# AlexZou14/Wave-Mamba

Hardware: AMD Instinct MI355X
Metric: UHD (3840x2160) images/sec fwd (higher is better)
Workload: dtype f32; 1 GPU; Wave-Mamba UHD-LL inference config (wf=32, n_l=[1,2,4], n_h=[1,1,2]), 1x3x2160x3840 reflect-padded to 2176x3840, seeded random init, one image per GPU per step, replicas (no collective); one forward at a time, its down-path high-frequency branches on side streams: True

## Files before the change

### include/wavemamba_hip.h

```cpp
#ifndef WAVEMAMBA_HIP_H
#define WAVEMAMBA_HIP_H

#include <stddef.h>
#include <stdint.h>

#ifdef __cplusplus
extern "C" {
#endif

#define WM_OK 0
#define WM_EINVAL (-1)
#define WM_ENULL (-2)
#define WM_EALIGN (-3)
#define WM_EWORKSPACE (-4)
#define WM_EUNSUPPORTED (-5)
#define WM_EHIP (-6)

#define WM_F32 0
#define WM_BF16 1

int wm_abi_version(void);
const char* wm_build_id(void);
const char* wm_strerror(int code);

// ... 52 lines not shown
                       int C, int plane_dtype, void* stream);
int wm_lfss_out_fwd(const void* fc, const float* tok1, const float* conv3_weight, const float* conv3_bias,
                    const float* skip_scale2, float* out, int out_nchw, int B, int64_t L, int C, int plane_dtype,
                    void* stream);
int wm_lfss_in_conv_fwd(const float* tok, int tok_nchw, const float* ln_w, const float* ln_b, float ln_eps,
                        const float* in_proj_weight, const float* conv_weight, const float* conv_bias, float* xc,
                        int B, int H, int W, int C, int plane_dtype, void* stream);
int wm_lfss_in_conv_band_rows(int B, int H, int W);
int wm_lfss_out_conv_fwd(const void* f, const float* conv2_weight, const float* conv2_bias, const float* tok1,
                         const float* conv3_weight, const float* conv3_bias, const float* skip_scale2, float* out,
                         int out_nchw, int B, int H, int W, int C, int plane_dtype, void* stream);

int wm_layernorm2d_fwd(const float* x, const float* weight, const float* bias, float eps, float* y,
                       int B, int64_t L, int C, void* stream);

size_t wm_gram_workspace_bytes(int B, int C, int64_t L);
int wm_gram_fwd(const float* X, const float* Y, float* G, float* nx, float* ny, void* workspace,
                size_t workspace_bytes, int B, int C, int64_t L, void* stream);

int wm_dwconv3x3_wgrad(const float* x, const float* gy, float* dW, float* db, int B, int C, int H, int W,
                       void* stream);
int wm_layernorm2d_bwd(const float* x, const float* weight, const float* gy, float eps, float* gx,
                       float* dweight, float* dbias, int B, int64_t L, int C, void* stream);


int wm_conv2d_select(int mode);
size_t wm_conv2d_wfrag_bytes(int Cout, int Cin, int ks);
int wm_conv2d_prep(const float* weight, void* wfrag, int Cout, int Cin, int ks, void* stream);
int wm_conv2d_ln_fwd(const float* x, const float* ln_weight, const float* ln_bias, float ln_eps, const void* wfrag, const float* bias,
                     const float* residual, float* y, int B, int Cin, int Cout, int H, int W, void* stream);
int wm_dwconv_conv1x1_fwd(const float* x, int64_t x_batch_stride, const float* dw_weight, const float* dw_bias, int act,
                          const void* wfrag, const float* bias, const float* residual, float* y, int B, int C, int Cout, int H,
                          int W, void* stream);
int wm_conv2d_f16_steps(const float* x, const float* weight, const float* bias, float* y, float* amax, void* wfrag, int B, int Cin,
                        int Cout, int H, int W, int ks, int dgrad, void* stream);
int wm_conv2d_fwd(const float* xa, const float* xb, const int* xb_index, const void* wfrag, const float* bias,
                  const float* gate, const float* residual, float* y, int B, int Ca, int Cb, int Cb_src, int Cout,
                  int H, int W, int ks, void* stream);
int wm_conv2d_gated_fwd(const float* xa, const float* xb, const int* xb_index, const void* wfrag3, const void* wfrag1,
                        const float* bias1, float* y, int B, int Ca, int Cb, int Cb_src, int Cout, int H, int W,
                        void* stream);
int wm_conv2d_dwt_fwd(const void* img, const void* wfrag, const float* bias, void* ll, void* hl, void* lh, void* hh, int B, int Cin,
                      int Cout, int H, int W, int dtype, void* stream);
int wm_idwt_conv2d_fwd(const void* low, const void* high, const void* wfrag, const float* bias, const float* residual, float* y, int B,
                       int Cin, int Cout, int H, int W, int dtype, void* stream);

size_t wm_ss2d_core_bwd_workspace_bytes(int B, int D, int H, int W, int N, int R);
int wm_ss2d_core_bwd(const float* x, const float* x_proj_weight, const float* dt_projs_weight,
                     const float* dt_projs_bias, const float* A_logs, const float* Ds, const float* dy_row_fwd,
                     const float* dy_row_rev, const float* dy_col_fwd, const float* dy_col_rev, float* dx,
                     float* dx_proj_weight, float* ddt_projs_weight, float* ddt_projs_bias, float* dA_logs, float* dDs,
                     void* workspace, size_t workspace_bytes, int B, int D, int H, int W, int N, int R, void* stream);

int wm_layernorm_tok_fwd(const float* x, const float* weight, const float* bias, float eps, float* y, int64_t T, int C,
                         void* stream);
int wm_layernorm_tok_bwd(const float* x, const float* weight, const float* gy, float eps, float* gx, float* dweight,
                         float* dbias, int64_t T, int C, void* stream);

int wm_image_pre_u8(const uint8_t* image, float* out, int h, int w, int Hp, int Wp, int swap_rb, void* stream);
int wm_image_post_u8(const float* in, uint8_t* image, int h, int w, int Hp, int Wp, int swap_rb, void* stream);

int wm_paired_patches_u8(const int64_t* table, float* lq, float* gt, int B, int P, int swap_rb, void* stream);

int wm_linear_wgrad(const float* gy, const float* x, float* dW, int64_t T, int O, int I, void* stream);
size_t wm_conv2d_wgrad_workspace_bytes(int B, int Cin, int Cout, int H, int W, int ks);
int wm_conv2d_wgrad(const float* gy, const float* x, float* dW, float* db, void* workspace, size_t workspace_bytes, int B, int Cin,
// ... 52 lines not shown
```

### wave_mamba_amd/_lib.py

```python
import ctypes
import os

HERE = os.path.dirname(os.path.abspath(__file__))
LIB_PATH = os.environ.get("WAVEMAMBA_HIP_LIB") or os.path.join(HERE, "libwavemamba_hip.so")

WM_F32, WM_BF16 = 0, 1
WM_OK, WM_EINVAL, WM_ENULL, WM_EALIGN, WM_EWORKSPACE, WM_EUNSUPPORTED, WM_EHIP = 0, -1, -2, -3, -4, -5, -6
WM_PROF_NKERNELS = 20
ABI_VERSION = 34

_c = ctypes
_p, _i, _i64, _sz = _c.c_void_p, _c.c_int, _c.c_int64, _c.c_size_t

SIGNATURES = {
    "wm_abi_version": (_i, []),
    "wm_build_id": (_c.c_char_p, []),
    "wm_strerror": (_c.c_char_p, [_i]),
    "wm_dwt2d_fwd": (_i, [_p] * 5 + [_i] * 5 + [_p]),
    "wm_dwt2d_bwd": (_i, [_p] * 5 + [_i] * 5 + [_p]),
    "wm_idwt2d_fwd": (_i, [_p] * 4 + [_i64] * 4 + [_p] + [_i] * 5 + [_p]),
    "wm_idwt2d_bwd": (_i, [_p] * 5 + [_i64] * 4 + [_i] * 5 + [_p]),
    "wm_selscan_fwd_workspace_bytes": (_sz, [_i] * 5),
    "wm_selscan_fwd": (_i, [_p] * 10 + [_p, _sz] + [_i] * 6 + [_p]),
    "wm_selscan_bwd_workspace_bytes": (_sz, [_i] * 5),
# ... 20 lines not shown
    "wm_dwconv3x3_wgrad": (_i, [_p] * 4 + [_i] * 4 + [_p]),
    "wm_layernorm2d_bwd": (_i, [_p, _p, _p, _c.c_float, _p, _p, _p, _i, _i64, _i, _p]),
    "wm_dwconv3x3_fwd": (_i, [_p] * 4 + [_i] * 6 + [_p]),
    "wm_layernorm_tok_fwd": (_i, [_p, _p, _p, _c.c_float, _p, _i64, _i, _p]),
    "wm_layernorm_tok_bwd": (_i, [_p, _p, _p, _c.c_float, _p, _p, _p, _i64, _i, _p]),
    "wm_image_pre_u8": (_i, [_p, _p, _i, _i, _i, _i, _i, _p]),
    "wm_image_post_u8": (_i, [_p, _p, _i, _i, _i, _i, _i, _p]),
    "wm_paired_patches_u8": (_i, [_p, _p, _p, _i, _i, _i, _p]),
    "wm_linear_wgrad": (_i, [_p, _p, _p, _i64, _i, _i, _p]),
    "wm_conv2d_wgrad_workspace_bytes": (_sz, [_i] * 6),
    "wm_conv2d_wgrad": (_i, [_p, _p, _p, _p, _p, _sz] + [_i] * 6 + [_p]),
    "wm_plane_sums": (_i, [_p, _p, _i, _i, _i, _i, _p]),
    "wm_psnr_ssim_y_workspace_bytes": (_sz, [_i] * 4),
    "wm_psnr_ssim_y_u8": (_i, [_p, _p] + [_i64] * 4 + [_i] * 5 + [_p, _p, _sz, _p]),
    "wm_y_channel_u8": (_i, [_p] + [_i64] * 4 + [_i] * 4 + [_p, _p]),
    "wm_l1_mean_fwd": (_i, [_p, _p, _p, _i64, _p]),
    "wm_l1_mean_bwd": (_i, [_p, _p, _p, _p, _i64, _p]),
    "wm_ssim_workspace_bytes": (_sz, [_i64, _i, _i]),
    "wm_ssim_mean_fwd": (_i, [_p] * 8 + [_sz, _i64, _i, _i, _p]),
    "wm_ssim_mean_bwd": (_i, [_p] * 7 + [_i64, _i, _i, _p]),
    "wm_gate_fwd": (_i, [_p] * 3 + [_i, _i] + [_i64] * 4 + [_p]),
    "wm_gate_bwd": (_i, [_p] * 5 + [_i, _i] + [_i64] * 6 + [_p]),
    "wm_scale_add_fwd": (_i, [_p] * 4 + [_i, _i, _i64, _p]),
    "wm_scale_add_bwd": (_i, [_p] * 5 + [_i, _i, _i64, _p]),
    "wm_match_index": (_i, [_p, _p, _p, _p, _i, _i, _p]),
    "wm_attn_fold": (_i, [_p] * 6 + [_i, _i, _i, _p]),
    "wm_skff_workspace_bytes": (_sz, [_i, _i]),
    "wm_skff_fwd": (_i, [_p] * 7 + [_p, _sz] + [_i] * 5 + [_p]),
    "wm_conv2d_wfrag_bytes": (_sz, [_i, _i, _i]),
    "wm_conv2d_prep": (_i, [_p, _p, _i, _i, _i, _p]),
    "wm_conv2d_fwd": (_i, [_p] * 8 + [_i] * 8 + [_p]),
    "wm_conv2d_ln_fwd": (_i, [_p, _p, _p, _c.c_float, _p, _p, _p, _p] + [_i] * 5 + [_p]),
    "wm_dwconv_conv1x1_fwd": (_i, [_p, _i64, _p, _p, _i, _p, _p, _p, _p] + [_i] * 5 + [_p]),
    "wm_patchify_conv_fwd": (_i, [_p] * 4 + [_i] * 6 + [_p]),
    "wm_conv2d_f16_steps": (_i, [_p] * 6 + [_i] * 7 + [_p]),
    "wm_conv2d_gated_fwd": (_i, [_p] * 7 + [_i] * 7 + [_p]),
    "wm_conv2d_dwt_fwd": (_i, [_p] * 7 + [_i] * 6 + [_p]),
    "wm_idwt_conv2d_fwd": (_i, [_p] * 6 + [_i] * 6 + [_p]),
    "wm_conv2d_select": (_i, [_i]),
    "wm_prof_enable": (None, [ctypes.c_uint]),
    "wm_prof_collect": (_i, [_c.POINTER(_i), _c.POINTER(_c.c_double)]),
    "wm_event_synchronize_relaxed": (_i, [_p]),
    "wm_zero_arena_register": (_i, [_p, _c.c_size_t]),
    "wm_zero_arena_unregister": (_i, [_p]),
}

_lib = None


class WaveMambaHipError(RuntimeError):
    pass


def load():
    global _lib
    if _lib is not None:
        return _lib
    if not os.path.exists(LIB_PATH):
        raise WaveMambaHipError(
            f"{LIB_PATH} not found: build it with `python -c 'import __graft_entry__ as g; g.build()'` "
            "(hipcc --offload-arch=gfx950). The Wave-Mamba hot path has no CPU or PyTorch fallback.")
    try:
        lib = ctypes.CDLL(LIB_PATH)
    except OSError as e:
        raise WaveMambaHipError(f"cannot load {LIB_PATH}: {e}") from e
    for name, (res, args) in SIGNATURES.items():
# ... 24 lines not shown
```

### wave_mamba_amd/archs/wavemamba_arch.py

```python
import math

import os

import torch
import torch.nn as nn
import torch.nn.functional as F

try:
    from .. import ops as _hip_ops
    from ..registry import ARCH_REGISTRY
except ImportError:
    import wave_mamba_amd.ops as _hip_ops
    from basicsr.utils.registry import ARCH_REGISTRY


class _OpsBackend:
    impl = _hip_ops


def _op(name):
    return getattr(_OpsBackend.impl, name, None)


def _needs_grad(module, *tensors):
# ... 44 lines not shown
        y = conv(x)
    if gate is not None:
        if train and _op("gate_act") and ops.gate_supported(gate, y):
            y = ops.gate_act(gate, y, "sigmoid")
        else:
            y = y * torch.sigmoid(gate)
    if residual is not None:
        y = y + residual
    return y


def _ps_conv(ps, img):
    ops = _OpsBackend.impl
    r, conv = ps[0].downscale_factor, ps[1]
    if _op("patchify_conv") and ops.patchify_conv_supported(img, conv.weight, r) and not _needs_grad(conv, img):
        return ops.patchify_conv(img, conv.weight, conv.bias, r)
    return _conv(conv, ps[0](img))


def _ln_conv(norm, conv, x):
    if norm is None:
        return _conv(conv, x)
    ops = _OpsBackend.impl
    if (_op("conv2d_ln") and ops.conv2d_ln_supported(x, conv.weight) and not _needs_grad(conv, x)
            and not _needs_grad(norm, x)):
        return ops.conv2d_ln(x, norm.weight, norm.bias, norm.eps, conv.weight, conv.bias)
    return _conv(conv, norm(x))


def _dw_pw_fused(x, dw_weight, pw_weight):
    ops = _OpsBackend.impl
    return bool(_op("dwconv_conv1x1") and ops.dwconv_conv1x1_supported(x, dw_weight, pw_weight)
                and _hip_ops._fuse_dw_pw_map(x.shape[0], x.shape[2], x.shape[3]))


def _conv_dwt_fused(conv, img):
    ops = _OpsBackend.impl
    return bool(_op("conv2d_dwt") and ops.conv2d_dwt_supported(img, conv.weight) and not _needs_grad(conv, img)
                and _hip_ops._fuse_conv_dwt_map(img.shape[0], img.shape[2], img.shape[3]))


def _conv_dwt(conv, img):
    if _conv_dwt_fused(conv, img):
        return _OpsBackend.impl.conv2d_dwt(img, conv.weight, conv.bias)
    return _conv(conv, img)


def _iwt_conv_fused(net, conv, low, out_like):
    ops = _OpsBackend.impl
    return bool(_op("iwt_conv2d") and ops.iwt_conv2d_supported(low, conv.weight) and not _needs_grad(net, low, out_like)
                and _hip_ops._fuse_iwt_conv_map(out_like.shape[0], out_like.shape[2], out_like.shape[3]))


def _cat_gathered(x, x2=None, x2_index=None):
    if x2 is None:
        return x
    if x2_index is not None:
        x2 = torch.gather(x2, 1, x2_index.long()[:, :, None, None].expand(-1, -1, x2.shape[2], x2.shape[3]))
    return torch.cat([x, x2], dim=1)


class DWT(nn.Module):

    def forward(self, x):
        return _OpsBackend.impl.dwt_init(x)

# ... 292 lines not shown
class Matching_transformation(nn.Module):
    def __init__(self, dim=32, match_factor=1, ffn_expansion_factor=1, bias=True):
        super().__init__()
        self.num_matching = int(dim / match_factor)
        self.channel = dim
        self.matching = Matching(dim=dim, match_factor=match_factor)
        self.paconv = PAConv(dim * 2)

    def forward(self, x, perception):
        idx = nearest_candidate_index(x.flatten(2), perception.flatten(2), self.num_matching)
        return self.paconv(x, perception, idx)


class FeedForward(nn.Module):

    def __init__(self, dim=32, match_factor=4, ffn_expansion_factor=1, bias=True, ffn_matching=True):
        super().__init__()
        self.num_matching = int(dim / match_factor)
        self.channel = dim
        self.matching = ffn_matching
        hidden = int(dim * ffn_expansion_factor)
        self.project_in = nn.Sequential(
            nn.Conv2d(dim, hidden, 1, bias=bias),
            nn.Conv2d(hidden, dim, kernel_size=3, stride=1, padding=1, groups=dim, bias=bias))
        if self.matching is True:
            self.matching_transformation = Matching_transformation(
                dim=dim, match_factor=match_factor, ffn_expansion_factor=ffn_expansion_factor, bias=bias)
        self.project_out = nn.Sequential(
            nn.Conv2d(dim, hidden, kernel_size=3, stride=1, padding=1, groups=dim, bias=bias),
            nn.GELU(),
            nn.Conv2d(hidden, dim, 1, bias=bias))

    def forward(self, x, perception, residual=None, norm=None):
        y = _dwconv(self.project_in[1], _ln_conv(norm, self.project_in[0], x))
        if perception is not None:
            y = self.matching_transformation(y, perception)
        dw, pw = self.project_out[0], self.project_out[2]
        if _dw_pw_fused(y, dw.weight, pw.weight) and not _needs_grad(dw, y, residual) and not _needs_grad(pw):
            return _OpsBackend.impl.dwconv_conv1x1(y, dw.weight, dw.bias, "gelu", pw.weight, pw.bias, residual=residual)
        return _conv(pw, _dwconv(dw, y, act="gelu"), residual=residual)


class CMTAttention(nn.Module):

    def __init__(self, dim, num_heads, match_factor=4, ffn_expansion_factor=1, scale_factor=8, bias=True,
                 attention_matching=True):
        super().__init__()
        self.num_heads = num_heads
        self.temperature = nn.Parameter(torch.ones(num_heads, 1, 1))
        self.qkv = nn.Conv2d(dim, dim * 3, kernel_size=1, bias=bias)
        self.qkv_dwconv = nn.Conv2d(dim * 3, dim * 3, kernel_size=3, stride=1, padding=1, groups=dim * 3,
                                    bias=bias)
        self.project_out = nn.Conv2d(dim, dim, kernel_size=1, bias=bias)
        self.matching = attention_matching
        if self.matching is True:
            self.matching_transformation = Matching_transformation(
                dim=dim, match_factor=match_factor, ffn_expansion_factor=ffn_expansion_factor, bias=bias)

    def qkv_of(self, x, norm=None):
        pre = _ln_conv(norm, self.qkv, x)
        dw = self.qkv_dwconv
        c = pre.shape[1] // 3
        ops = _OpsBackend.impl
        if (pre.shape[0] == 1 and _op("attn_fold") and _op("dwconv3x3") and ops.dwconv3x3_supported(pre)
                and _dw_pw_fused(pre[:, 2 * c:], dw.weight[2 * c:], self.project_out.weight) and not _needs_grad(self, pre)):
            return ops.dwconv3x3(pre[:, :2 * c], dw.weight[:2 * c], None if dw.bias is None else dw.bias[:2 * c]), pre
        return _dwconv(dw, pre)

    def forward(self, x, perception, residual=None, qkv=None, norm=None):
        qkv = self.qkv_of(x, norm) if qkv is None else qkv
        pre = None
        if isinstance(qkv, tuple):
            qk, pre = qkv
            (q, k), v = qk.chunk(2, dim=1), None
        else:
            q, k, v = qkv.chunk(3, dim=1)
        x = k
        b, c, h, w = x.shape
        dw = self.qkv_dwconv
        dw_v = (dw.weight[2 * c:], None if dw.bias is None else dw.bias[2 * c:])

        def value():
            return v if pre is None else _OpsBackend.impl.dwconv3x3(pre[:, 2 * c:], *dw_v)
        if self.matching is True:
            q = self.matching_transformation(q, perception)
        heads = self.num_heads
        q = q.reshape(b * heads, c // heads, h * w)
        k = k.reshape(b * heads, c // heads, h * w)
        ops = _OpsBackend.impl
        train_gram = _needs_grad(None, q, k)
        if _op("gram") and ops.gram_supported(q, k) and (not train_gram or _op("gram_train")):
            G, nq, nk = ops.gram_train(q, k) if train_gram else ops.gram(q.contiguous(), k.contiguous())
            if (_op("attn_fold") and ops.attn_fold_supported(x, self.project_out.weight, heads)
                    and not _needs_grad(self)):
                wf = ops.attn_fold(G, nq, nk, self.temperature.reshape(heads), self.project_out.weight, b, heads)
                if pre is not None:
                    return ops.dwconv_conv1x1(pre[:, 2 * c:], *dw_v, "none", wf[0].view(c, c, 1, 1), self.project_out.bias,
                                              residual=residual, dynamic_weight=True)
                outs = [ops.conv2d(v[i:i + 1], wf[i].view(c, c, 1, 1), self.project_out.bias,
                                   residual=None if residual is None else residual[i:i + 1], dynamic_weight=True)
                        for i in range(b)]
                return outs[0] if b == 1 else torch.cat(outs, 0)
            scale = nq.clamp_min(1e-24).sqrt().unsqueeze(2) * nk.clamp_min(1e-24).sqrt().unsqueeze(1)
            attn = (G / scale).reshape(b, heads, c // heads, c // heads)
        else:
            qn = F.normalize(q.reshape(b, heads, c // heads, h * w), dim=-1)
            kn = F.normalize(k.reshape(b, heads, c // heads, h * w), dim=-1)
            attn = qn @ kn.transpose(-2, -1)
        attn = (attn * self.temperature).softmax(dim=-1)
        return _conv(self.project_out, (attn @ value().reshape(b, heads, c // heads, h * w)).reshape(b, c, h, w), residual=residual)


class HFEBlock(nn.Module):

    def __init__(self, dim=48, num_heads=1, match_factor=4, ffn_expansion_factor=1, bias=True,
                 attention_matching=True, ffn_matching=True, ffn_restormer=False):
        super().__init__()
        if ffn_restormer:
            raise NotImplementedError("ffn_restormer=True is never instantiated by the reference UNet")
        self.dim = dim
        self.norm1 = LayerNorm2d(dim)
        self.attn = CMTAttention(dim=dim, num_heads=num_heads, match_factor=match_factor,
                                 ffn_expansion_factor=ffn_expansion_factor, bias=bias,
                                 attention_matching=attention_matching)
        self.norm2 = LayerNorm2d(dim)
        self.ffn_restormer = ffn_restormer
        self.ffn = FeedForward(dim=dim, match_factor=match_factor, ffn_expansion_factor=ffn_expansion_factor,
                               bias=bias, ffn_matching=ffn_matching)
        self.LayerNorm = LayerNorm2d(dim)

# ... 260 lines not shown
```

### wave_mamba_amd/csrc/conv.hip

```cpp
#include "host_common.h"
#include "conv2d.hip.h"
#include "conv2d_ws.hip.h"
#include "patchify.hip.h"
#include "dw_pw.hip.h"

using namespace wm;

template <int KS, int RW, int MT, bool G1X1 = false, bool F16 = false, bool LNIN = false>
static int conv2d_launch(const wm::Conv2dArgs& a, int B, hipStream_t st) {
    constexpr int PAD = KS / 2;
    constexpr int smem = ((4 * RW + 2 * PAD) * (wm::kCvTW + 2 * PAD) * 4 + (KS * KS + (G1X1 ? 1 : 0)) * MT * 2 * 64) * 16;
    static bool configured[64] = {};
    if (smem > 65536) {
        const int rc = wm::lds_optin((const void*)wm::conv2d_mfma_kernel<KS, RW, MT, G1X1, F16, LNIN>, smem, configured);
        if (rc) return rc;
    }
    const int ntiles = ((a.W + wm::kCvTW - 1) / wm::kCvTW) * ((a.H + 4 * RW - 1) / (4 * RW));
    const dim3 grid((unsigned)(((ntiles + 7) / 8) * 8), (unsigned)B);
    hipLaunchKernelGGL((wm::conv2d_mfma_kernel<KS, RW, MT, G1X1, F16, LNIN>), grid, dim3(256), smem, st, a);
    return launch_status();
}

#ifndef WM_CONV_WS_RW2
#define WM_CONV_WS_RW2 4
#endif
#ifndef WM_CONV_WS_RW1
#define WM_CONV_WS_RW1 4
#endif
#ifndef WM_CONV_WS_RWG
#define WM_CONV_WS_RWG 2
#endif
#ifndef WM_CONV_WS_NPW1
#define WM_CONV_WS_NPW1 4
#endif
static std::atomic<int> g_conv_select{0};
static int conv_select_mode() { return g_conv_select.load(std::memory_order_relaxed); }
static bool conv_ws_enabled(const wm::Conv2dArgs& a, int B, int th) {
// ... 151 lines not shown

int wm_dwconv_conv1x1_fwd(const float* x, int64_t x_batch_stride, const float* dw_weight, const float* dw_bias, int act,
                          const void* wfrag, const float* bias, const float* residual, float* y, int B, int C, int Cout, int H,
                          int W, void* stream) {
    if (B < 0 || C <= 0 || Cout <= 0 || H < 0 || W < 0 || x_batch_stride < 0) return WM_EINVAL;
    if (act != 0 && act != 2) return WM_EINVAL;
    if (C != 32 || Cout != 32) return WM_EUNSUPPORTED;
    if (B == 0 || H == 0 || W == 0) return WM_OK;
    if (!x || !dw_weight || !wfrag || !y) return WM_ENULL;
    if ((long long)H * W >= (1ll << 26)) return WM_EUNSUPPORTED;
    if (B > 1 && x_batch_stride < (long long)C * H * W) return WM_EINVAL;
    if (!aligned16(wfrag)) return WM_EALIGN;
    hipStream_t st = (hipStream_t)stream;
    DwPwArgs a;
    a.x = x; a.xbs = x_batch_stride; a.dw_w = dw_weight; a.dw_b = dw_bias; a.wfrag = (const uint4*)wfrag; a.bias = bias;
    a.res = residual; a.y = y; a.H = H; a.W = W;
    a.nstrips = (W + kCvTW - 1) / kCvTW;
    a.rows = 4;
    for (int rows = 16; rows > 4; rows >>= 1)
        if ((long long)B * a.nstrips * ((H + rows - 1) / rows) >= 1024) { a.rows = rows; break; }
    a.nbands = (H + a.rows - 1) / a.rows;
    a.nwalks = (long long)B * a.nbands * a.nstrips;
    const long long nblocks = ((a.nwalks + 3) / 4 + 7) / 8 * 8;
    if (nblocks >= (1ll << 31)) return WM_EUNSUPPORTED;
    const dim3 grid((unsigned)nblocks);
    ProfScope ps(14, st);
    if (act == 2) {
        if (residual) hipLaunchKernelGGL((dw_pw_kernel<true, true>), grid, dim3(256), 0, st, a);
        else hipLaunchKernelGGL((dw_pw_kernel<true, false>), grid, dim3(256), 0, st, a);
    } else {
        if (residual) hipLaunchKernelGGL((dw_pw_kernel<false, true>), grid, dim3(256), 0, st, a);
        else hipLaunchKernelGGL((dw_pw_kernel<false, false>), grid, dim3(256), 0, st, a);
    }
    return launch_status();
}

static int conv2d_fwd_f16(const float* x, const void* wfrag, const float* amax, const float* bias, float* y, int B, int Cin, int Cout,
                          int H, int W, int ks, void* stream) {
    if (B < 0 || Cin <= 0 || Cout <= 0 || H < 0 || W < 0) return WM_EINVAL;
    if (ks != 1 && ks != 3) return WM_EUNSUPPORTED;
    if (B == 0 || H == 0 || W == 0) return WM_OK;
    if (!x || !wfrag || !y || !amax) return WM_ENULL;
    if (B > 65535 || (long long)H * W >= (1ll << 31)) return WM_EUNSUPPORTED;
    if (!aligned16(wfrag)) return WM_EALIGN;
    hipStream_t st = (hipStream_t)stream;
    Conv2dArgs a;
    a.xa = x; a.xb = nullptr; a.xb_idx = nullptr; a.wfrag = (const uint4*)wfrag;
    a.bias = bias; a.gate = nullptr; a.res = nullptr; a.y = y; a.wfrag1 = nullptr; a.bias1 = nullptr;
    a.Ca = Cin; a.Cb = 0; a.Cbsrc = 0; a.Cout = Cout; a.H = H; a.W = W;
    a.nch = (Cin + 15) / 16; a.mtot = (Cout + 31) / 32; a.amax = amax; a.ln_w = nullptr; a.ln_b = nullptr; a.ln_eps = 0.0f;
    ProfScope ps(ks == 3 ? 13 : 14, st);
    for (int mb = 0; mb < a.mtot;) {
        a.mbase = mb;
        const int left = a.mtot - mb;
        int rc;
        if (ks == 3) {
            if (conv_ws_enabled(a, B, 8)) {
                if (left >= 2) { rc = conv2d_ws_launch<WM_CONV_WS_RW2, 2, false, false, 4, true>(a, B, st); mb += 2; }
                else { rc = conv2d_ws_launch<WM_CONV_WS_RW1, 1, false, false, WM_CONV_WS_NPW1, true>(a, B, st); mb += 1; }
            } else if (left >= 2) { rc = conv2d_launch<3, 4, 2, false, true>(a, B, st); mb += 2; }
            else { rc = conv2d_launch<3, WM_CONV_RW1, 1, false, true>(a, B, st); mb += 1; }
        } else {
            if (left >= 3) { rc = conv2d_launch<1, 2, 3, false, true>(a, B, st); mb += 3; }
            else if (left == 2) { rc = conv2d_launch<1, 4, 2, false, true>(a, B, st); mb += 2; }
            else { rc = conv2d_launch<1, 4, 1, false, true>(a, B, st); mb += 1; }
        }
// ... 120 lines not shown
```

### wave_mamba_amd/csrc/dwconv.hip.h

```cpp
#pragma once
#include <hip/hip_runtime.h>
#include "haar.hip.h"

namespace wm {

__device__ __forceinline__ float dpp_from_lower_lane(float own_if_first, float v) {
    return __builtin_bit_cast(float, __builtin_amdgcn_update_dpp(__builtin_bit_cast(int, own_if_first), __builtin_bit_cast(int, v),
                                                                 0x138 , 0xf, 0xf, false));
}
__device__ __forceinline__ float dpp_from_upper_lane(float own_if_last, float v) {
    return __builtin_bit_cast(float, __builtin_amdgcn_update_dpp(__builtin_bit_cast(int, own_if_last), __builtin_bit_cast(int, v),
                                                                 0x130 , 0xf, 0xf, false));
}

constexpr int kDwRows = 16;

__device__ __forceinline__ float silu_f(float v) { return v / (1.0f + __expf(-v)); }

__device__ __forceinline__ float gelu_erf(float v) { return 0.5f * v * (1.0f + erff(v * 0.70710678118654752440f)); }

__device__ __forceinline__ float dw_taps3(float acc, const float* w, const float* r) {
    acc = fmaf(w[0], r[0], acc); acc = fmaf(w[1], r[1], acc); acc = fmaf(w[2], r[2], acc);
    return acc;
}
__device__ __forceinline__ float dw_taps9(float bias, const float* w, const float* r0, const float* r1, const float* r2) {
    return dw_taps3(dw_taps3(dw_taps3(bias, w, r0), w + 3, r1), w + 6, r2);
}

template <int ACT , bool VEC, typename TP = float, int LPR = 64>
__global__ __launch_bounds__(256) void dwconv3x3_kernel(const TP* __restrict__ x,
                                                        const float* __restrict__ wgt,
                                                        const float* __restrict__ bias,
                                                        TP* __restrict__ y, int C, int H, int W,
                                                        long long planes, int rows, int flip) {
    constexpr int PPW = 64 / LPR;
    const int lane = threadIdx.x;
    const int cl = lane & (LPR - 1);
    const int cg = blockIdx.x * LPR + cl;
    const int h0 = (blockIdx.y * 4 + threadIdx.y) * rows;
    for (long long pg = blockIdx.z; pg * PPW < planes; pg += gridDim.z) {
        const long long plane_raw = pg * PPW + (LPR == 64 ? 0 : lane / LPR);
        const bool pok = plane_raw < planes;
        const long long plane = pok ? plane_raw : planes - 1;
        const int c = (int)(plane % C);
        float k[9];
// ... 222 lines not shown
```

### wave_mamba_amd/csrc/lfss_mfma.hip.h

```cpp
#pragma once
#include <hip/hip_runtime.h>
#include "haar.hip.h"
#include "dwconv.hip.h"

#ifndef WM_LFSS_MID_WAVES
#define WM_LFSS_MID_WAVES 3
#endif
#ifndef WM_LFSS_MID_RZ_WAVES
#define WM_LFSS_MID_RZ_WAVES 2
#endif
#ifndef WM_LFSS_IN_WAVES
#define WM_LFSS_IN_WAVES 4
#endif
#ifndef WM_LFSS_MID_YB_RZ
#define WM_LFSS_MID_YB_RZ 16
#endif
#ifndef WM_LFSS_OUT_TILE
#define WM_LFSS_OUT_TILE 8
#endif

namespace wm {

typedef float lfss_v16f __attribute__((ext_vector_type(16)));

__device__ __forceinline__ float silu_fast(float v) {
    return v * __builtin_amdgcn_rcpf(1.0f + __builtin_amdgcn_exp2f(v * -1.4426950408889634f));
}
__device__ __forceinline__ float xhalf_sum(float v) { return v + __shfl_xor(v, 32); }
__device__ __forceinline__ lfss_v16f mfma32(float a, float b, lfss_v16f acc) { return __builtin_amdgcn_mfma_f32_32x32x2f32(a, b, acc, 0, 0, 0); }

template <typename TP>
__device__ __forceinline__ __amdgpu_buffer_rsrc_t raw_rsrc(const TP* p, int bytes) {
    return __builtin_amdgcn_make_buffer_rsrc(const_cast<TP*>(p), 0, bytes, 0x00020000);
}

inline int lfss_groups_per_wave(long long ngroups, int slots) {
    const long long rounds = (ngroups + 8LL * slots - 1) / (8LL * slots);
    long long gpw = (ngroups + rounds * slots - 1) / (rounds * slots);
    return (int)(gpw < 1 ? 1 : gpw);
}
__device__ __forceinline__ void group_pos(long long g, int ngl, long long& b, long long& p0) { b = g / ngl; p0 = (g - b * ngl) * 64; }

__device__ __forceinline__ void load_tile32(const float* __restrict__ src, bool nchw, long long b, long long pq,
                                            long long L, int h, float (&v)[16]) {
#pragma unroll
    for (int gq = 0; gq < 4; ++gq) {
        const int row0 = 8 * gq + 4 * h;
        if (nchw) {
            const float* tp = src + (b * 32 + row0) * L + pq;
            v[4 * gq] = tp[0]; v[4 * gq + 1] = tp[L]; v[4 * gq + 2] = tp[2 * L]; v[4 * gq + 3] = tp[3 * L];
        } else {
            const float4 t = *reinterpret_cast<const float4*>(src + (b * L + pq) * 32 + row0);
            v[4 * gq] = t.x; v[4 * gq + 1] = t.y; v[4 * gq + 2] = t.z; v[4 * gq + 3] = t.w;
        }
    }
}
__device__ __forceinline__ void store_tile32(float* __restrict__ dst, bool nchw, long long b, long long pos,
                                             long long L, int h, const float (&v)[16]) {
#pragma unroll
    for (int gq = 0; gq < 4; ++gq) {
        const int row0 = 8 * gq + 4 * h;
        if (nchw) {
            float* tp = dst + (b * 32 + row0) * L + pos;
            tp[0] = v[4 * gq]; tp[L] = v[4 * gq + 1]; tp[2 * L] = v[4 * gq + 2]; tp[3 * L] = v[4 * gq + 3];
        } else {
            *reinterpret_cast<float4*>(dst + (b * L + pos) * 32 + row0) =
                make_float4(v[4 * gq], v[4 * gq + 1], v[4 * gq + 2], v[4 * gq + 3]);
// ... 692 lines not shown
```

### wave_mamba_amd/ops.py

```python
import os
import weakref

import torch
import torch.nn.functional as F

from . import _lib
from ._lib import WM_BF16, WM_F32, check


def _stream():
    return torch.cuda.current_stream().cuda_stream


def _require_cuda(name, *tensors):
    for t in tensors:
        if t is not None and not t.is_cuda:
            raise RuntimeError(
                f"{name}: expected a CUDA (ROCm) tensor, got device '{t.device}'. The Wave-Mamba hot "
                "path is HIP-only (dwt_init / iwt_init / selective_scan_fn alone have a CPU twin, for inputs that are ALL "
                "on the CPU); nothing falls back to the CPU.")


def _dtype_code(t, name):
    if t.dtype == torch.float32:
# ... 1040 lines not shown
_FUSE_DW_PW = True
_FUSE_DW_PW_MIN_POSITIONS = 272 * 480


def _fuse_dw_pw_map(B, H, W):
    return _FUSE_DW_PW and B > 0 and _FUSE_DW_PW_MIN_POSITIONS <= H * W < (1 << 26)


def dwconv_conv1x1_supported(x, dw_weight, weight):
    return (x.is_cuda and x.dim() == 4 and x.shape[1] == 32 and tuple(dw_weight.shape) == (32, 1, 3, 3)
            and tuple(weight.shape) == (32, 32, 1, 1) and all(t.dtype == torch.float32 for t in (x, dw_weight, weight)))


def dwconv_conv1x1(x, dw_weight, dw_bias, act, weight, bias=None, residual=None, dynamic_weight=False):
    _require_cuda("dwconv_conv1x1", x, dw_weight, dw_bias, weight, bias, residual)
    if not dwconv_conv1x1_supported(x, dw_weight, weight):
        raise NotImplementedError("dwconv_conv1x1: fp32, 32 -> 32 channels, (32, 1, 3, 3) depth-wise and (32, 32, 1, 1) dense weights")
    if act not in ("none", "gelu"):
        raise ValueError(f"dwconv_conv1x1: act must be 'none' or 'gelu', got {act!r}")
    B, C, H, W = x.shape
    if residual is not None and (tuple(residual.shape) != (B, 32, H, W) or residual.dtype != torch.float32):
        raise RuntimeError(f"dwconv_conv1x1: residual must be float32 {(B, 32, H, W)}, got {tuple(residual.shape)}")
    if tuple(x.stride()[1:]) != (H * W, W, 1) or (B > 1 and x.stride(0) < C * H * W):
        x = x.contiguous()
    frag = _conv2d_wfrag(weight, cache=not dynamic_weight)
    y = torch.empty((B, 32, H, W), dtype=torch.float32, device=x.device)
    _launch(x.device, "wm_dwconv_conv1x1_fwd", x, x.stride(0) if B > 1 else C * H * W, _w(dw_weight),
            None if dw_bias is None else _w(dw_bias), {"none": 0, "gelu": 2}[act], frag,
            None if bias is None else bias.detach().contiguous(), None if residual is None else residual.contiguous(), y,
            B, C, 32, H, W)
    return y


_FUSE_CONV_DWT = True
_FUSE_CONV_DWT_MIN_POSITIONS = 1088 * 1920


def _fuse_conv_dwt_map(B, H, W):
    return _FUSE_CONV_DWT and B == 1 and H * W >= _FUSE_CONV_DWT_MIN_POSITIONS


def conv2d_dwt_supported(x, weight):
    return (x.is_cuda and x.dim() == 4 and weight.dim() == 4 and tuple(weight.shape) == (32, x.shape[1], 3, 3)
            and x.dtype == torch.float32 and weight.dtype == torch.float32 and x.shape[2] % 2 == 0 and x.shape[3] % 2 == 0
            and x.shape[0] <= 65535 and max(32, x.shape[1]) * x.shape[2] * x.shape[3] * 4 < 2 ** 32)


def conv2d_dwt(x, weight, bias=None):
    _require_cuda("conv2d_dwt", x, weight, bias)
    if not conv2d_dwt_supported(x, weight):
        raise NotImplementedError("conv2d_dwt: fp32, a (32, Cin, 3, 3) weight, even H and W, the wave-specialised 3x3 kernel's limits")
    B, Cin, H, W = x.shape
    x = x.contiguous()
    frag = _conv2d_wfrag(weight)
    outs = [torch.empty((B, 32, H // 2, W // 2), dtype=torch.float32, device=x.device) for _ in range(4)]
    rc = _launch(x.device, "wm_conv2d_dwt_fwd", x, frag, None if bias is None else bias.detach().contiguous(), *outs, B, Cin, 32, H, W,
                 WM_F32, status=True)
    if rc == _lib.WM_EUNSUPPORTED:
        return dwt_init(conv2d(x, weight, bias))
    check(rc, "wm_conv2d_dwt_fwd")
    return tuple(outs)


_FUSE_IWT_CONV = True
_FUSE_IWT_CONV_MIN_POSITIONS = 1088 * 1920

# ... 364 lines not shown
```

Measured before the change: 35.21 images/s.

## Fuse LayerNorm, 1x1 conv and depthwise 3x3 into one row-walking kernel

Adds a HIP kernel that applies channel LayerNorm, a 32-input 1x1 conv on MFMA, and a 3x3 depthwise conv in a single pass. Each wave walks a column strip of row bands and keeps the depthwise partial sums in registers across rows. It is used for the FFN project_in (32->32) and for the attention qkv head, where the q/k channels get the depthwise conv and v is left raw for the later dw+pw fusion. This removes the intermediate full-resolution tensor write and re-read, plus a kernel launch, per block. The cost is halo rows recomputed at band edges and higher register pressure. It is gated by resolution thresholds.

```diff
diff --git a/include/wavemamba_hip.h b/include/wavemamba_hip.h
--- a/include/wavemamba_hip.h
+++ b/include/wavemamba_hip.h
@@ -108,6 +108,9 @@
 int wm_dwconv_conv1x1_fwd(const float* x, int64_t x_batch_stride, const float* dw_weight, const float* dw_bias, int act,
                           const void* wfrag, const float* bias, const float* residual, float* y, int B, int C, int Cout, int H,
                           int W, void* stream);
+int wm_ln_conv1x1_dwconv_fwd(const float* x, const float* ln_weight, const float* ln_bias, float ln_eps, const void* wfrag,
+                             const float* bias, const float* dw_weight, const float* dw_bias, float* y, int B, int Cin, int Cout,
+                             int Cdw, int H, int W, int band_rows, void* stream);
 int wm_conv2d_f16_steps(const float* x, const float* weight, const float* bias, float* y, float* amax, void* wfrag, int B, int Cin,
                         int Cout, int H, int W, int ks, int dgrad, void* stream);
 int wm_conv2d_fwd(const float* xa, const float* xb, const int* xb_index, const void* wfrag, const float* bias,
diff --git a/wave_mamba_amd/_lib.py b/wave_mamba_amd/_lib.py
--- a/wave_mamba_amd/_lib.py
+++ b/wave_mamba_amd/_lib.py
@@ -76,6 +76,7 @@
     "wm_conv2d_fwd": (_i, [_p] * 8 + [_i] * 8 + [_p]),
     "wm_conv2d_ln_fwd": (_i, [_p, _p, _p, _c.c_float, _p, _p, _p, _p] + [_i] * 5 + [_p]),
     "wm_dwconv_conv1x1_fwd": (_i, [_p, _i64, _p, _p, _i, _p, _p, _p, _p] + [_i] * 5 + [_p]),
+    "wm_ln_conv1x1_dwconv_fwd": (_i, [_p, _p, _p, _c.c_float, _p, _p, _p, _p, _p] + [_i] * 7 + [_p]),
     "wm_patchify_conv_fwd": (_i, [_p] * 4 + [_i] * 6 + [_p]),
     "wm_conv2d_f16_steps": (_i, [_p] * 6 + [_i] * 7 + [_p]),
     "wm_conv2d_gated_fwd": (_i, [_p] * 7 + [_i] * 7 + [_p]),
diff --git a/wave_mamba_amd/archs/wavemamba_arch.py b/wave_mamba_amd/archs/wavemamba_arch.py
--- a/wave_mamba_amd/archs/wavemamba_arch.py
+++ b/wave_mamba_amd/archs/wavemamba_arch.py
@@ -100,6 +100,15 @@
     ops = _OpsBackend.impl
     return bool(_op("dwconv_conv1x1") and ops.dwconv_conv1x1_supported(x, dw_weight, pw_weight)
                 and _hip_ops._fuse_dw_pw_map(x.shape[0], x.shape[2], x.shape[3]))
+
+
+def _pw_dw_fused(norm, conv, dw_weight, x):
+    ops = _OpsBackend.impl
+    if norm is None or not (_op("conv2d_ln") and _op("ln_conv1x1_dwconv") and ops.conv2d_ln_supported(x, conv.weight)):
+        return False
+    head = ops.ln_conv1x1_dwconv_supported(x, conv.weight, dw_weight, dw_weight.shape[0])
+    return bool(head and _hip_ops._fuse_pw_dw_map(x.shape[0], x.shape[2], x.shape[3], head)
+                and not _needs_grad(conv, x) and not _needs_grad(norm))
 
 
 def _conv_dwt_fused(conv, img):
@@ -458,7 +467,12 @@
             nn.Conv2d(hidden, dim, 1, bias=bias))
 
     def forward(self, x, perception, residual=None, norm=None):
-        y = _dwconv(self.project_in[1], _ln_conv(norm, self.project_in[0], x))
+        pw_in, dw_in = self.project_in
+        if _pw_dw_fused(norm, pw_in, dw_in.weight, x) and not _needs_grad(dw_in):
+            y = _OpsBackend.impl.ln_conv1x1_dwconv(x, norm.weight, norm.bias, norm.eps, pw_in.weight, pw_in.bias, dw_in.weight,
+                                                   dw_in.bias, dw_in.weight.shape[0])
+        else:
+            y = _dwconv(dw_in, _ln_conv(norm, pw_in, x))
         if perception is not None:
             y = self.matching_transformation(y, perception)
         dw, pw = self.project_out[0], self.project_out[2]
@@ -484,13 +498,18 @@
                 dim=dim, match_factor=match_factor, ffn_expansion_factor=ffn_expansion_factor, bias=bias)
 
     def qkv_of(self, x, norm=None):
+        dw = self.qkv_dwconv
+        c = self.qkv.weight.shape[0] // 3
+        ops = _OpsBackend.impl
+        dw_qk = (dw.weight[:2 * c], None if dw.bias is None else dw.bias[:2 * c])
+        if (x.shape[0] == 1 and _op("attn_fold") and _op("dwconv3x3") and _pw_dw_fused(norm, self.qkv, dw_qk[0], x)
+                and _dw_pw_fused(x, dw.weight[2 * c:], self.project_out.weight) and not _needs_grad(self, x)):
+            y = ops.ln_conv1x1_dwconv(x, norm.weight, norm.bias, norm.eps, self.qkv.weight, self.qkv.bias, *dw_qk, 2 * c)
+            return y[:, :2 * c], y[:, 2 * c:]
         pre = _ln_conv(norm, self.qkv, x)
-        dw = self.qkv_dwconv
-        c = pre.shape[1] // 3
-        ops = _OpsBackend.impl
         if (pre.shape[0] == 1 and _op("attn_fold") and _op("dwconv3x3") and ops.dwconv3x3_supported(pre)
                 and _dw_pw_fused(pre[:, 2 * c:], dw.weight[2 * c:], self.project_out.weight) and not _needs_grad(self, pre)):
-            return ops.dwconv3x3(pre[:, :2 * c], dw.weight[:2 * c], None if dw.bias is None else dw.bias[:2 * c]), pre
+            return ops.dwconv3x3(pre[:, :2 * c], *dw_qk), pre[:, 2 * c:]
         return _dwconv(dw, pre)
 
     def forward(self, x, perception, residual=None, qkv=None, norm=None):
@@ -507,7 +526,7 @@
         dw_v = (dw.weight[2 * c:], None if dw.bias is None else dw.bias[2 * c:])
 
         def value():
-            return v if pre is None else _OpsBackend.impl.dwconv3x3(pre[:, 2 * c:], *dw_v)
+            return v if pre is None else _OpsBackend.impl.dwconv3x3(pre, *dw_v)
         if self.matching is True:
             q = self.matching_transformation(q, perception)
         heads = self.num_heads
@@ -521,7 +540,7 @@
                     and not _needs_grad(self)):
                 wf = ops.attn_fold(G, nq, nk, self.temperature.reshape(heads), self.project_out.weight, b, heads)
                 if pre is not None:
-                    return ops.dwconv_conv1x1(pre[:, 2 * c:], *dw_v, "none", wf[0].view(c, c, 1, 1), self.project_out.bias,
+                    return ops.dwconv_conv1x1(pre, *dw_v, "none", wf[0].view(c, c, 1, 1), self.project_out.bias,
                                               residual=residual, dynamic_weight=True)
                 outs = [ops.conv2d(v[i:i + 1], wf[i].view(c, c, 1, 1), self.project_out.bias,
                                    residual=None if residual is None else residual[i:i + 1], dynamic_weight=True)
diff --git a/wave_mamba_amd/csrc/conv.hip b/wave_mamba_amd/csrc/conv.hip
--- a/wave_mamba_amd/csrc/conv.hip
+++ b/wave_mamba_amd/csrc/conv.hip
@@ -3,6 +3,7 @@
 #include "conv2d_ws.hip.h"
 #include "patchify.hip.h"
 #include "dw_pw.hip.h"
+#include "pw_dw.hip.h"
 
 using namespace wm;
 
@@ -220,6 +221,33 @@
         if (residual) hipLaunchKernelGGL((dw_pw_kernel<false, true>), grid, dim3(256), 0, st, a);
         else hipLaunchKernelGGL((dw_pw_kernel<false, false>), grid, dim3(256), 0, st, a);
     }
+    return launch_status();
+}
+
+int wm_ln_conv1x1_dwconv_fwd(const float* x, const float* ln_weight, const float* ln_bias, float ln_eps, const void* wfrag,
+                             const float* bias, const float* dw_weight, const float* dw_bias, float* y, int B, int Cin, int Cout,
+                             int Cdw, int H, int W, int band_rows, void* stream) {
+    if (B < 0 || Cin <= 0 || Cout <= 0 || Cdw <= 0 || H < 0 || W < 0 || band_rows < 0) return WM_EINVAL;
+    const bool qkv = Cout == 96 && Cdw == 64, pin = Cout == 32 && Cdw == 32;
+    if (Cin != 32 || !(qkv || pin)) return WM_EUNSUPPORTED;
+    if (B == 0 || H == 0 || W == 0) return WM_OK;
+    if (!x || !ln_weight || !ln_bias || !wfrag || !dw_weight || !y) return WM_ENULL;
+    if ((long long)H * W >= (1ll << 25)) return WM_EUNSUPPORTED;
+    if (!aligned16(wfrag)) return WM_EALIGN;
+    hipStream_t st = (hipStream_t)stream;
+    PwDwArgs a;
+    a.x = x; a.ln_w = ln_weight; a.ln_b = ln_bias; a.ln_eps = ln_eps; a.wfrag = (const uint4*)wfrag; a.bias = bias;
+    a.dw_w = dw_weight; a.dw_b = dw_bias; a.y = y; a.H = H; a.W = W;
+    a.nstrips = (W + kPwDwCols - 1) / kPwDwCols;
+    a.rows = band_rows ? band_rows : ((long long)B * a.nstrips * ((H + 7) / 8) >= 2048 ? 8 : 4);
+    a.nbands = (H + a.rows - 1) / a.rows;
+    a.nwalks = (long long)B * a.nbands * a.nstrips;
+    const long long nblocks = ((a.nwalks + 3) / 4 + 7) / 8 * 8;
+    if (nblocks >= (1ll << 31)) return WM_EUNSUPPORTED;
+    const dim3 grid((unsigned)nblocks);
+    ProfScope ps(14, st);
+    if (qkv) hipLaunchKernelGGL((pw_dw_kernel<3, 2>), grid, dim3(256), 0, st, a);
+    else hipLaunchKernelGGL((pw_dw_kernel<1, 1>), grid, dim3(256), 0, st, a);
     return launch_status();
 }
 
diff --git a/wave_mamba_amd/csrc/dwconv.hip.h b/wave_mamba_amd/csrc/dwconv.hip.h
--- a/wave_mamba_amd/csrc/dwconv.hip.h
+++ b/wave_mamba_amd/csrc/dwconv.hip.h
@@ -11,6 +11,11 @@
 __device__ __forceinline__ float dpp_from_upper_lane(float own_if_last, float v) {
     return __builtin_bit_cast(float, __builtin_amdgcn_update_dpp(__builtin_bit_cast(int, own_if_last), __builtin_bit_cast(int, v),
                                                                  0x130 , 0xf, 0xf, false));
+}
+
+template <typename TP>
+__device__ __forceinline__ __amdgpu_buffer_rsrc_t raw_rsrc(const TP* p, int bytes) {
+    return __builtin_amdgcn_make_buffer_rsrc(const_cast<TP*>(p), 0, bytes, 0x00020000);
 }
 
 constexpr int kDwRows = 16;
diff --git a/wave_mamba_amd/csrc/lfss_mfma.hip.h b/wave_mamba_amd/csrc/lfss_mfma.hip.h
--- a/wave_mamba_amd/csrc/lfss_mfma.hip.h
+++ b/wave_mamba_amd/csrc/lfss_mfma.hip.h
@@ -28,11 +28,6 @@
 }
 __device__ __forceinline__ float xhalf_sum(float v) { return v + __shfl_xor(v, 32); }
 __device__ __forceinline__ lfss_v16f mfma32(float a, float b, lfss_v16f acc) { return __builtin_amdgcn_mfma_f32_32x32x2f32(a, b, acc, 0, 0, 0); }
-
-template <typename TP>
-__device__ __forceinline__ __amdgpu_buffer_rsrc_t raw_rsrc(const TP* p, int bytes) {
-    return __builtin_amdgcn_make_buffer_rsrc(const_cast<TP*>(p), 0, bytes, 0x00020000);
-}
 
 inline int lfss_groups_per_wave(long long ngroups, int slots) {
     const long long rounds = (ngroups + 8LL * slots - 1) / (8LL * slots);
diff --git a/wave_mamba_amd/csrc/pw_dw.hip.h b/wave_mamba_amd/csrc/pw_dw.hip.h
--- /dev/null
+++ b/wave_mamba_amd/csrc/pw_dw.hip.h
@@ -0,0 +1,180 @@
+#pragma once
+#include "conv2d.hip.h"
+#include "dwconv.hip.h"
+#include "dw_pw.hip.h"
+
+namespace wm {
+
+struct PwDwArgs {
+    const float* x;
+    const float* ln_w;
+    const float* ln_b;
+    float ln_eps;
+    const uint4* wfrag;
+    const float* bias;
+    const float* dw_w;
+    const float* dw_b;
+    float* y;
+    int H, W;
+    int nstrips, nbands, rows;
+    long long nwalks;
+};
+
+constexpr int kPwDwCols = kCvTW - 2;
+
+template <int NT, int NDW>
+__global__ __launch_bounds__(256, 2) void pw_dw_kernel(const PwDwArgs a) {
+    static_assert(NDW >= 1 && NDW <= NT, "the depth-wise convolution reads the first NDW row tiles");
+    constexpr int C = 32;
+    __shared__ uint4 s_A[2 * NT * 2 * 64];
+    __shared__ __attribute__((aligned(16))) float s_tap[NDW * 32 * 12];
+    __shared__ __attribute__((aligned(16))) float s_bias[NT * 32];
+    __shared__ __attribute__((aligned(16))) float s_ln[2 * 2 * 16];
+    const int lane = threadIdx.x & 63, px = lane & 31, kh = lane >> 5;
+    const int wv = __builtin_amdgcn_readfirstlane(threadIdx.x >> 6);
+    const long long blk = (long long)(blockIdx.x & 7) * (gridDim.x >> 3) + (blockIdx.x >> 3);
+    const bool live = blk * 4 + wv < a.nwalks;
+    const long long wk = live ? blk * 4 + wv : a.nwalks - 1;
+    const int strip = (int)(wk % a.nstrips);
+    const long long wb = wk / a.nstrips;
+    const int band = (int)(wb % a.nbands);
+    const long long b = wb / a.nbands;
+    const int H = a.H, W = a.W, HW = H * W;
+    const float* __restrict__ xb = a.x + b * C * HW;
+    float* __restrict__ yb = a.y + b * (NT * 32) * HW;
+
+    const int col = strip * kPwDwCols - 1 + px;
+    const bool colin = col >= 0 && col < W;
+    const bool st_ok = px >= 1 && px <= kPwDwCols && col < W;
+    const unsigned xoff = 4u * (8 * kh * HW + min(max(col, 0), W - 1));
+    const unsigned plane_bytes = 4u * HW, nrec = 32u * plane_bytes;
+    const unsigned lane_off = 4u * (4 * kh * HW + min(col, W - 1));
+    __amdgpu_buffer_rsrc_t rs[NT];
+#pragma unroll
+    for (int m = 0; m < NT; ++m) rs[m] = raw_rsrc(yb + (long long)m * 32 * HW, (int)nrec);
+
+    const int r0 = band * a.rows, r_end = min(H, r0 + a.rows);
+    auto load_row = [&](int rho, float (&nx)[16]) {
+        const unsigned ro = 4u * (min(max(rho, 0), H - 1) * W);
+#pragma unroll
+        for (int c = 0; c < 16; ++c) nx[c] = *dwpw_at(xb + (16 * (c >> 3) + (c & 7)) * HW, xoff + ro);
+    };
+    float nxa[16], nxb[16];
+    load_row(r0 - 1, nxa);
+    __builtin_amdgcn_sched_barrier(0);
+    load_row(r0, nxb);
+    __builtin_amdgcn_sched_barrier(0);
+
+    for (int i = threadIdx.x; i < NT * 32; i += 256) {
+        const int r = i & 15;
+        s_bias[i] = a.bias ? a.bias[32 * (i >> 5) + 4 * ((i >> 4) & 1) + (r & 3) + 8 * (r >> 2)] : 0.0f;
+    }
+    for (int i = threadIdx.x; i < NDW * 32 * 12; i += 256) {
+        const int c = i / 12, t = i - c * 12;
+        s_tap[i] = t < 9 ? a.dw_w[c * 9 + t] : (t == 9 && a.dw_b) ? a.dw_b[c] : 0.0f;
+    }
+    if (threadIdx.x < 64) {
+        const int h = threadIdx.x >> 5, e = threadIdx.x & 15, c = 16 * (e >> 3) + 8 * h + (e & 7);
+        s_ln[threadIdx.x] = (threadIdx.x & 16) ? a.ln_b[c] : a.ln_w[c];
+    }
+    for (int i = threadIdx.x; i < 2 * NT * 2 * 64; i += 256) s_A[i] = a.wfrag[i];
+    __syncthreads();
+    if (!live) return;
+
+    float p0[NDW * 16], p1[NDW * 16];
+#pragma unroll
+    for (int q = 0; q < NDW * 16; ++q) p0[q] = p1[q] = 0.0f;
+
+    auto step = [&](int rho, float (&nx)[16]) {
+        int lo = lane, ko = kh;
+        asm volatile("" : "+v"(lo), "+v"(ko));
+        Frag16 Bh[2], Bl[2];
+        {
+            float f[32];
+#pragma unroll
+            for (int c = 0; c < 16; ++c) {
+                const auto r = __builtin_amdgcn_permlane32_swap(__float_as_uint(nx[c]), __float_as_uint(nx[c]), false, false);
+                f[16 * (c >> 3) + (c & 7)] = __uint_as_float(r[0]);
+                f[16 * (c >> 3) + 8 + (c & 7)] = __uint_as_float(r[1]);
+            }
+            float mean = 0.0f;
+#pragma unroll
+            for (int c = 0; c < 32; ++c) mean += f[c];
+            mean *= (1.0f / 32.0f);
+            float var = 0.0f;
+#pragma unroll
+            for (int c = 0; c < 32; ++c) { const float q = f[c] - mean; var = fmaf(q, q, var); }
+            const float rstd = 1.0f / sqrtf(var * (1.0f / 32.0f) + a.ln_eps);
+            const float4* l4 = reinterpret_cast<const float4*>(s_ln + 32 * ko);
+#pragma unroll
+            for (int q = 0; q < 4; ++q) {
+                const float4 wq = l4[q], bq = l4[4 + q];
+                const float lw[4] = {wq.x, wq.y, wq.z, wq.w}, lb[4] = {bq.x, bq.y, bq.z, bq.w};
+#pragma unroll
+                for (int j = 0; j < 4; ++j) {
+                    const int c = 4 * q + j;
+                    cv_split<false>(fmaf((nx[c] - mean) * rstd, lw[j], lb[j]), Bh[c >> 3], Bl[c >> 3], c & 7);
+                }
+            }
+        }
+        load_row(rho + 2, nx);
+        __builtin_amdgcn_sched_barrier(0);
+        const bool rowin = rho >= 0 && rho < H;
+        const bool keep = colin && rowin;
+        const bool orow_dw = rho - 1 >= r0 && rho - 1 < r_end, orow_pw = rho >= r0 && rho < r_end;
+        const unsigned voff_dw = (st_ok && orow_dw) ? lane_off + 4u * ((rho - 1) * W) : nrec;
+        const unsigned voff_pw = (st_ok && orow_pw) ? lane_off + 4u * (rho * W) : nrec;
+#pragma unroll
+        for (int m = 0; m < NT; ++m) {
+            f32x16_t acc;
+#pragma unroll
+            for (int i = 0; i < 16; ++i) acc[i] = 0.0f;
+#pragma unroll
+            for (int cc = 0; cc < 2; ++cc) {
+                Frag16 Ah, Al;
+                Ah.u = s_A[((cc * NT + m) * 2 + 0) * 64 + lo];
+                Al.u = s_A[((cc * NT + m) * 2 + 1) * 64 + lo];
+                acc = cv_mfma<false>(Ah, Bh[cc], acc);
+                acc = cv_mfma<false>(Ah, Bl[cc], acc);
+                acc = cv_mfma<false>(Al, Bh[cc], acc);
+            }
+            const float4* b4 = reinterpret_cast<const float4*>(s_bias + 32 * m + 16 * ko);
+            const float* tap = s_tap + (32 * m + 4 * ko) * 12;
+#pragma unroll
+            for (int q = 0; q < 4; ++q) {
+                const float4 bq = b4[q];
+                const float bv[4] = {bq.x, bq.y, bq.z, bq.w};
+#pragma unroll
+                for (int j = 0; j < 4; ++j) {
+                    const int i = 4 * q + j, ch = (i & 3) + 8 * (i >> 2);
+                    float v = acc[i] + bv[j];
+                    if (m < NDW) {
+                        asm("" : "+v"(v));
+                        const float xm = keep ? v : 0.0f;
+                        const float t3[3] = {dpp_from_lower_lane(0.0f, xm), xm, dpp_from_upper_lane(0.0f, xm)};
+                        const float4* t4 = reinterpret_cast<const float4*>(tap + ch * 12);
+                        const float4 ta = t4[0], tb = t4[1], tc = t4[2];
+                        const float t[10] = {ta.x, ta.y, ta.z, ta.w, tb.x, tb.y, tb.z, tb.w, tc.x, tc.y};
+                        const int pq = 16 * (m < NDW ? m : 0) + i;
+                        v = dw_taps3(p1[pq], t + 6, t3);
+                        p1[pq] = dw_taps3(p0[pq], t + 3, t3);
+                        p0[pq] = dw_taps3(t[9], t, t3);
+                        asm volatile("" : "+v"(p0[pq]), "+v"(p1[pq]));
+                    }
+                    __builtin_amdgcn_raw_buffer_store_b32(__float_as_uint(v), rs[m], (int)(m < NDW ? voff_dw : voff_pw),
+                                                          (int)(ch * plane_bytes), 0);
+                    if (m < NDW) __builtin_amdgcn_sched_barrier(0);
+                }
+            }
+            __builtin_amdgcn_sched_barrier(0);
+        }
+    };
+
+#pragma unroll 1
+    for (int rho = r0 - 1; rho <= r_end; rho += 2) {
+        step(rho, nxa);
+        step(rho + 1, nxb);
+    }
+}
+
+}
diff --git a/wave_mamba_amd/ops.py b/wave_mamba_amd/ops.py
--- a/wave_mamba_amd/ops.py
+++ b/wave_mamba_amd/ops.py
@@ -1096,6 +1096,38 @@
     return y
 
 
+_FUSE_PW_DW = True
+_FUSE_PW_DW_MIN_POSITIONS = {"qkv": 544 * 960, "project_in": 272 * 480}
+_PW_DW_HEADS = {"qkv": (96, 64), "project_in": (32, 32)}
+
+
+def _fuse_pw_dw_map(B, H, W, head):
+    floor = _FUSE_PW_DW_MIN_POSITIONS[head]
+    return bool(_FUSE_PW_DW and B > 0 and floor <= H * W < (1 << 25))
+
+
+def ln_conv1x1_dwconv_supported(x, weight, dw_weight, n_dw):
+    if not (x.is_cuda and x.dim() == 4 and x.shape[1] == 32 and weight.dim() == 4 and tuple(weight.shape[1:]) == (32, 1, 1)
+            and tuple(dw_weight.shape) == (n_dw, 1, 3, 3) and all(t.dtype == torch.float32 for t in (x, weight, dw_weight))):
+        return None
+    return next((h for h, form in _PW_DW_HEADS.items() if form == (weight.shape[0], n_dw)), None)
+
+
+def ln_conv1x1_dwconv(x, ln_w, ln_b, eps, weight, bias, dw_weight, dw_bias, n_dw, band_rows=0):
+    _require_cuda("ln_conv1x1_dwconv", x, ln_w, ln_b, weight, bias, dw_weight, dw_bias)
+    if ln_conv1x1_dwconv_supported(x, weight, dw_weight, n_dw) is None:
+        raise NotImplementedError("ln_conv1x1_dwconv: fp32, 32 input channels, (Cout, n_dw) = (96, 64) or (32, 32)")
+    B, C, H, W = x.shape
+    cout = weight.shape[0]
+    x = x.contiguous()
+    frag = _conv2d_wfrag(weight)
+    y = torch.empty((B, cout, H, W), dtype=torch.float32, device=x.device)
+    _launch(x.device, "wm_ln_conv1x1_dwconv_fwd", x, _w(ln_w), _w(ln_b), float(eps), frag,
+            None if bias is None else bias.detach().contiguous(), _w(dw_weight), None if dw_bias is None else _w(dw_bias), y,
+            B, C, cout, n_dw, H, W, int(band_rows))
+    return y
+
+
 _FUSE_CONV_DWT = True
 _FUSE_CONV_DWT_MIN_POSITIONS = 1088 * 1920
 
```

Result: faster. 35.73 images/s, median of 6 (+1.5%).
